# shwetabhardwaj44/EfficientVideoClassification_Youtube8M

Measured on AMD Instinct MI355X. Metric: frames/sec (whole node) H-LSTM teacher+student B=256x300x1152; GAP@20, higher is better.
Workload: dtype bf16; 1 GPU; HierarchicalLstmModel teacher_student every_n=10, lstm_cells=1024x2, MoE(2), batch 256 x 300 x 1152 per GPU; global_batch=256, frames_per_video=300, parallelism=dp1, num_frames=U{120..300}

## Files before the change

### efficientvideoclassification_youtube8m_amd/_lib.py

```python
from __future__ import annotations

import ctypes as C
import os

_HERE = os.path.dirname(os.path.abspath(__file__))
LIB_PATH = os.environ.get("EVC_LIB", os.path.join(_HERE, "libevc_hip.so"))

vp, i32, i64, f32 = C.c_void_p, C.c_int, C.c_int64, C.c_float

SIGNATURES = {
    "evc_check_device": [i32],
    "evc_l2norm_chunk_fwd": [vp, vp, vp, i32, i32, i32, i32, vp, i32, i32, vp, i32, vp, vp, i32, vp, i32, vp, i32, vp],
    "evc_sort_rows_by_len": [vp, i32, i32, vp, vp, vp, vp],
    "evc_frame_counts": [vp, i32, i32, i32, i32, i32, i32, vp, vp, vp, vp],
    "evc_gemm_nt": [vp, i64, vp, i64, vp, i64, i32, i32, i32, vp, i32, i32, vp],
    "evc_gemm_nt_sqnorm": [vp, i64, vp, i64, vp, i64, i32, i32, i32, vp, f32, vp, vp, i64, vp],
    "evc_gemm_tn": [vp, i64, vp, i64, vp, i64, i32, i32, i32, i32, i32, vp],
    "evc_gemm_tn2": [vp, i64, vp, i64, i32, vp, i64, i32, i32, vp, i64, i32, i32, i32, i32, vp],
    "evc_gemm_tn2_rows": [vp, i64, vp, i64, i32, vp, i64, i32, i32, vp, i64, i32, i32, i32, vp, i32, i32, vp],
    "evc_gemm_tn2_slabs": [vp, i64, vp, i64, i32, vp, i64, i32, i32, vp, i64, i64, i32, i32, i32, i32, vp],
    "evc_sum_slabs": [vp, i64, i32, i32, i32, i64, vp, i64, i32, vp],
    "evc_colsum_bf16": [vp, i64, i32, i32, i32, vp, vp],
    "evc_colsum_bf16_det": [vp, i64, i32, i32, i32, vp, vp, i32, vp],
    "evc_lstm_layer_fwd": [vp, vp, vp, vp, i32, i32, i32, i32, i32, vp, vp, vp, vp, i64, vp, vp, vp, vp, vp],
    "evc_lstm_layer_fwd_hp": [vp, vp, i64, vp, i64, vp, vp, i32, i32, i32, i32, vp, vp, vp, vp, vp, i64, vp, vp, vp],
    "evc_gemm_nt_split": [vp, i64, vp, i64, vp, i64, i32, i32, i32, vp, vp],
    "evc_cast_f32_to_f16_wide": [vp, i64, i32, i32, i32, i32, i32, vp, vp],
    "evc_cast_f32_to_bf16_wide": [vp, i64, i32, i32, vp, i64, i32, vp],
    "evc_lstm_layer_fwd_f16": [vp, i64, vp, vp, vp, i32, i32, i32, i32, vp, i32, vp, vp, vp, i64, vp, vp, vp, vp, vp],
    "evc_lstm_layer_fwd_f16_fp8lo": [vp, i64, i32, i64, i32, vp, vp, i32, i32, vp, vp, i32, i32, i32, vp, vp, vp, vp, i64, vp, vp, vp, vp, vp, vp, i32, vp],
    "evc_l2norm_chunk_int": [vp, vp, i32, i32, i32, i32, vp, i32, i32, vp, vp, vp, vp, vp, vp, i32, vp, i32, vp],
    "evc_lstm_level2_fwd_high": [vp, i64, i32, i64, i32, vp, vp, i32, i32, vp, vp, vp, i32, vp, i64, vp, vp, i32, i32, i32, vp, vp, vp, vp, vp, vp, vp, vp, i64,
                                 vp, vp, vp, vp, vp, vp, vp],
    "evc_lstm_layer_fwd_f16_dith": [vp, i64, i32, i64, i32, vp, i64, vp, i64, i32, vp, vp, i32, i32, i32, vp, vp, vp, vp, i64, vp, vp, vp, vp, vp],
    "evc_cast_f32_to_f16_dither": [vp, i64, i32, i64, C.c_uint32, vp, i64, i64, vp],
    "evc_lstm_stack2_fwd_f16_fp8lo": [vp, i32, vp, vp, vp, vp, vp, i32, i32, vp, vp, i32, i32, i32, i32, vp, vp, vp, vp, vp, vp, vp, vp, vp, i64, vp, vp, vp, vp, vp],
    "evc_cast_f32_to_fp8_lo": [vp, i64, i32, i32, i32, i32, i32, vp, i64, vp],
    "evc_cast_f32_to_fp8_lohi": [vp, i64, i32, i32, i32, i32, i32, vp, i64, vp],
    "evc_lstm_layer_bwd": [vp, vp, i32, i32, i32, i32, vp, vp, vp, vp, i64, vp, vp, vp, vp, vp, vp, vp, vp, vp],
    "evc_transpose_to_bf16": [vp, i32, i64, i32, i32, vp, i64, i32, i32, vp],
    "evc_cast_f32_to_bf16": [vp, i64, i32, i32, vp, i64, vp],
    "evc_cast_f32_to_f16": [vp, i64, i32, i32, vp, i64, vp],
    "evc_cast_f32_to_bf16_split": [vp, i64, i32, i32, vp, vp, i64, vp],
    "evc_rowsum_bf16": [vp, i64, i32, i32, vp, vp],
    "evc_lstm_stack2_fwd_f16": [vp, i32, vp, i32, vp, vp, vp, vp, i32, i32, i32, i32, vp, vp, vp, vp, vp, vp, vp, vp, vp, i64, vp, vp, vp, vp, vp],
    "evc_cast_f32_to_f16_segs": [vp, i64, i32, i32, i32, vp, vp],
    "evc_cast_f32_to_f16_wlo": [vp, i64, i32, i32, i32, vp, vp],
    "evc_lstm_level2_fwd": [vp, vp, vp, vp, vp, vp, i32, i32, i32, i32, vp, vp, vp, vp, vp, vp, i64, vp, vp, vp, vp, vp, vp, vp],
# ... 118 lines not shown
```

### efficientvideoclassification_youtube8m_amd/csrc/evc_gemm.hip

```cpp
#include "gemm_shared.h"

template <class Cfg, bool F16 = false, bool FP8 = false>
__global__ __launch_bounds__(Cfg::NT) void gemm_nt_kernel(GemmOperands p, StoreParams s, int tiles_m, int tiles_n) {
  static_assert(!FP8 || (F16 && is_v3<Cfg>::value), "the e4m3 tail rides behind f16 stages of the 64-wide ring loop");
  const int nwg = tiles_m * tiles_n;
  int bid = blockIdx.x, split = 0;
  if (s.splits > 1) {
    split = bid / nwg;
    bid -= split * nwg;
    const int k0 = split * s.ksteps_per_split;
    const int kstep = (is_v2<Cfg>::value && !is_v3<Cfg>::value) ? 32 : 64;
    p.A1 += (long)k0 * kstep;
    p.B += (long)k0 * kstep;
    p.nk1 = min(s.ksteps_per_split, p.nk1 - k0);
    if constexpr (FP8) {
      const int k8 = split * s.ksteps8_per_split;
      p.A3 += (long)k8 * 128;
      p.B8 += (long)k8 * 128;
      p.nk3 = min(s.ksteps8_per_split, p.nk3 - k8);
    }
  }
  const int id = xcd_remap(bid, nwg);
  int tm, tn;
  tile_of(id, tiles_m, tiles_n, tm, tn, s.splits > 1 ? patch_rows(nwg, tiles_n) : 8);
// ... 296 lines not shown
  GemmOperands p;
  p.A1 = (const bf16_t*)A16; p.lda1 = lda; p.nk1 = 0; p.A2 = p.A1; p.lda2 = lda; p.nk2 = 0;
  p.B = (const bf16_t*)B16; p.ldb = ldb; p.group_stride = 0; p.M = M; p.Nu = N;
  p.A1lo = p.A2lo = p.Blo = nullptr;
  p.A3 = A8; p.lda3 = lda8; p.A4 = A8; p.lda4 = lda8; p.B8 = B8; p.ldb8 = ldb8; p.scale8_exp = scale_exp;
  p.amax_ws = amax_ws; p.a8_hi_exp = a8_hi_exp;
  StoreParams s{C, ldc, M, N, bias, 0, 0, 1, 0};
  hipStream_t st = (hipStream_t)stream;
  if (M <= 512) {
    const int tiles = ceil_div(M, 256) * ceil_div(N, 64), nk16 = K16 / 64, nk8 = K8 / 128;
    int splits = 1;
    while (!evc_deterministic() && splits < 16 && tiles * splits * 2 <= 256 && nk16 % (splits * 2) == 0 && nk8 % (splits * 2) == 0 &&
           nk16 / (splits * 2) >= 4 && nk8 / (splits * 2) >= 4)
      splits *= 2;
    if (splits > 1) EVC_CHECK_HIP(hipMemset2DAsync(C, ldc * sizeof(float), 0, (size_t)N * sizeof(float), M, st));
    launch_gemm_f16_fp8<TileCfg3<256, 1, 64, 2, 4, 4>>(p, s, K16, K8, splits, st);
  } else {
    launch_gemm_f16_fp8<TileCfg3<256, 1, 256, 2, 4, 2>>(p, s, K16, K8, 1, st);
  }
  EVC_LAUNCH_CHECK();
  return EVC_OK;
}
extern "C" int evc_gemm_nt_f16_fp8(const evc_f16* A16, int64_t lda, const uint8_t* A8, int64_t lda8, const evc_f16* B16, int64_t ldb,
                                   const uint8_t* B8, int64_t ldb8, float* C, int64_t ldc, int M, int N, int K16, int K8, int scale_exp,
                                   const float* bias, void* stream) {
  return gemm_nt_f16_fp8_impl(A16, lda, A8, lda8, B16, ldb, B8, ldb8, C, ldc, M, N, K16, K8, scale_exp, nullptr, 0, bias, stream);
}
extern "C" int evc_gemm_nt_f16_fp8_dyn(const evc_f16* A16, int64_t lda, const uint8_t* A8, int64_t lda8, const evc_f16* B16, int64_t ldb,
                                       const uint8_t* B8, int64_t ldb8, float* C, int64_t ldc, int M, int N, int K16, int K8, int scale_exp,
                                       const float* amax_ws, int a8_hi_exp, const float* bias, void* stream) {
  EVC_REQUIRE(amax_ws && a8_hi_exp >= -30 && a8_hi_exp <= 30, EVC_ERR_BAD_ARG, "evc_gemm_nt_f16_fp8_dyn: amax_ws=%p a8_hi_exp=%d", (const void*)amax_ws, a8_hi_exp);
  return gemm_nt_f16_fp8_impl(A16, lda, A8, lda8, B16, ldb, B8, ldb8, C, ldc, M, N, K16, K8, scale_exp, amax_ws, a8_hi_exp, bias, stream);
}
```

### efficientvideoclassification_youtube8m_amd/csrc/gemm_core.h

```cpp
#pragma once
#include "evc_common.h"
#include <type_traits>

template <int BM_, int G_, int BU_, int WR_, int WC_>
struct TileCfg {
  static constexpr int BM = BM_, G = G_, BU = BU_, BN = G_ * BU_, WR = WR_, WC = WC_;
  static constexpr int WM = BM / WR, WU = BU / WC, MI = WM / 16, NI = WU / 16;
  static constexpr int NT = 64 * WR * WC;
  static constexpr int BK = 64;
  static constexpr int A_BYTES = BM * 128, B_BYTES = BN * 128, STAGE_BYTES = A_BYTES + B_BYTES;
  static constexpr int LDS_BYTES = 2 * STAGE_BYTES;
  static constexpr int ACH = BM * 8 / NT, BCH = BN * 8 / NT;
  static_assert(WM % 16 == 0 && WU % 16 == 0, "wave tile must be a multiple of 16x16");
  static_assert((BM * 8) % NT == 0 && (BN * 8) % NT == 0, "staging must divide evenly");
};

struct GemmOperands {
  const bf16_t* A1; long lda1; int nk1;
  const bf16_t* A2; long lda2; int nk2;
  const bf16_t* B;  long ldb;
  long group_stride;
  int M;
  int Nu;
  const bf16_t* A1lo; const bf16_t* A2lo; const bf16_t* Blo;
  const bf16_t* B2 = nullptr;
  const uint8_t* A3 = nullptr; long lda3 = 0; int nk3 = 0;
  const uint8_t* A4 = nullptr; long lda4 = 0; int nk4 = 0;
  const uint8_t* B8 = nullptr; long ldb8 = 0;
  int scale8_exp = 0;
  const float* amax_ws = nullptr; int a8_hi_exp = 0;
  const float* row_scale = nullptr; const float* col_add = nullptr; float g2_add = 0.f; long b8_gap = 0;
#ifdef EVC_STAMPS
  int stamp_slot = 0;
#endif
};

__device__ __forceinline__ int xcd_remap(int bid, int nwg) {
  const int xcd = bid & 7, q = nwg >> 3, r = nwg & 7;
  const int base = (xcd < r) ? xcd * (q + 1) : r * (q + 1) + (xcd - r) * q;
  return base + (bid >> 3);
}

__device__ __forceinline__ void tile_of(int id, int tiles_m, int tiles_n, int& tm, int& tn, const int GROUP_M = 8) {
  const int per_group = GROUP_M * tiles_n;
  const int g = id / per_group, r = id - g * per_group;
  const int first_m = g * GROUP_M;
  const int rows = min(tiles_m - first_m, GROUP_M);
  tm = first_m + r % rows;
  tn = r / rows;
}

__device__ __forceinline__ int patch_rows(int nwg, int tiles_n) {
  const int per = max(1, nwg >> 3);
  int gm = 1;
  while (gm * gm * 4 <= per) gm <<= 1;
  while (gm < per && per / gm > tiles_n) gm <<= 1;
  return min(gm, 8);
}

template <class Cfg, bool SWAP = false, bool INIT = true, bool F16 = false>
__device__ __forceinline__ void gemm_mainloop(const GemmOperands& p, const int m0, const int u0, char* lds,
                                              f32x4 (&acc)[Cfg::MI][Cfg::G][Cfg::NI]) {
  const int tid = threadIdx.x;
  const int lane = tid & 63;
// ... 135 lines not shown
```

### efficientvideoclassification_youtube8m_amd/csrc/gemm_core_v2.h

```cpp
#pragma once
#include "gemm_core.h"
#include <type_traits>

constexpr int LOOP_PRODUCER = 1, LOOP_DMA_FIRST = 2, LOOP_NO_PRIO = 4, LOOP_F16 = 8, LOOP_FP8_TAIL = 16;
constexpr int LOOP_B_NT = 64;
constexpr int LOOP_ROW_SCALE = 128;
constexpr int LOOP_MODE_DEFAULT = 0;

template <int BM_, int G_, int BU_, int WR_, int WC_, int STAGES_ = 5, bool PIPE_ = true>
struct TileCfg2 {
  static constexpr int BM = BM_, G = G_, BU = BU_, BN = G_ * BU_, WR = WR_, WC = WC_;
  static constexpr int WM = BM / WR, WU = BU / WC, MI = WM / 16, NI = WU / 16;
  static constexpr int NT = 64 * WR * WC;
  static constexpr int BK = 32, STAGES = STAGES_;
  static constexpr bool PIPE = PIPE_;
  static constexpr int A_BYTES = BM * 64, B_BYTES = BN * 64, STAGE_BYTES = A_BYTES + B_BYTES;
  static constexpr int ACH = (BM * 4 + NT - 1) / NT, BCH = (BN * 4 + NT - 1) / NT;
  static constexpr int PER = ACH + BCH;
  static constexpr bool RAGGED = (BM * 4) % NT != 0 || (BN * 4) % NT != 0;
  static constexpr int DUMMY_OFF = STAGES * STAGE_BYTES;
  static constexpr int LDS_BYTES = DUMMY_OFF + (RAGGED ? 1024 : 0);
  static_assert(WM % 16 == 0 && WU % 16 == 0, "wave tile must be a multiple of 16x16");
  static_assert(BM % 16 == 0 && BN % 16 == 0 && (NT / 4) % 16 == 0, "staging rows per round must keep (row>>2)&3 fixed");
  static_assert(LDS_BYTES <= 160 * 1024, "exceeds the 160 KiB LDS of a CU");
};

__device__ __forceinline__ int swz64(int row) { return (0xD2 >> (2 * ((row >> 2) & 3))) & 3; }

template <int N>
__device__ __forceinline__ void wait_vmcnt() {
  asm volatile("s_waitcnt vmcnt(%0)" ::"n"(N > 63 ? 63 : N) : "memory");
}

template <class Cfg, bool SWAP = false, bool INIT = true, int MODE = LOOP_MODE_DEFAULT>
__device__ __forceinline__ void gemm_mainloop_v2(const GemmOperands& p, const int m0, const int u0, char* lds,
                                                 f32x4 (&acc)[Cfg::MI][Cfg::G][Cfg::NI]) {
  const int tid = threadIdx.x;
  const int lane = tid & 63;
  const int wave = __builtin_amdgcn_readfirstlane(tid >> 6);
// ... 237 lines not shown
```

### efficientvideoclassification_youtube8m_amd/csrc/gemm_core_v3.h

```cpp
#pragma once
#include "gemm_core_v2.h"

#ifdef EVC_STAMPS
static __device__ unsigned long long evc_stamps[8][512][8];
#define EVC_STAMP(slot, k) do { if (threadIdx.x == 0 && blockIdx.x < 512) evc_stamps[(slot) & 7][blockIdx.x][k] = __builtin_amdgcn_s_memrealtime(); } while (0)
#else
#define EVC_STAMP(slot, k) do { } while (0)
#endif
typedef int v4i_t __attribute__((ext_vector_type(4)));
typedef int v8i_t __attribute__((ext_vector_type(8)));

template <int BM_, int G_, int BU_, int WR_, int WC_, int STAGES_ = 4, int MIP_ = 0>
struct TileCfg3 {
  static constexpr int BM = BM_, G = G_, BU = BU_, BN = G_ * BU_, WR = WR_, WC = WC_;
  static constexpr bool UNEVEN = MIP_ > 0;
  static constexpr int MIP = UNEVEN ? MIP_ : BM / WR / 16, MIC = UNEVEN ? BM / 16 - MIP_ : MIP;
  static constexpr int MI = MIP > MIC ? MIP : MIC, WM = UNEVEN ? MI * 16 : BM / WR, ROW1 = UNEVEN ? MIP * 16 : WM;
  static constexpr int WU = BU / WC, NI = WU / 16;
  static_assert(!UNEVEN || (WR == 2 && WC == 4 && BM % 16 == 0 && MIC > 0), "uneven split: two wave rows of four waves (wave row 0 = the producers)");
  static constexpr int NT = 64 * WR * WC;
  static constexpr int BK = 64, STAGES = STAGES_;
  static constexpr bool PIPE = true;
  static constexpr int A_BYTES = BM * 128, B_BYTES = BN * 128, STAGE_BYTES = A_BYTES + B_BYTES;
  static constexpr bool RAGGED = (BM / 8) % (NT / 64) != 0 || (BN / 8) % (NT / 64) != 0 || (BM / 8) % 4 != 0 || (BN / 8) % 4 != 0;
// ... 5 lines not shown
};

template <class Cfg, bool SWAP = false, bool INIT = true, int MODE = LOOP_MODE_DEFAULT, int PHASE = 0>
__device__ __forceinline__ void gemm_mainloop_v3(const GemmOperands& p, const int m0, const int u0, char* lds,
                                                 f32x4 (&acc)[Cfg::MI][Cfg::G][Cfg::NI]) {
  const int tid = threadIdx.x;
  const int lane = tid & 63;
  const int wave = __builtin_amdgcn_readfirstlane(tid >> 6);
  const int wr = wave / Cfg::WC, wc = wave % Cfg::WC;

  if (INIT && PHASE != 1) {
#pragma unroll
    for (int mi = 0; mi < Cfg::MI; ++mi)
#pragma unroll
      for (int g = 0; g < Cfg::G; ++g)
#pragma unroll
        for (int ni = 0; ni < Cfg::NI; ++ni) acc[mi][g][ni] = f32x4{0.f, 0.f, 0.f, 0.f};
  }
  constexpr bool FP8 = (MODE & LOOP_FP8_TAIL) != 0;
  const int nkf = p.nk1 + p.nk2;
  const int nk = nkf + (FP8 ? p.nk3 + p.nk4 : 0);
  if (nk == 0) return;

  const int lc8 = ((lane & 7) ^ (lane >> 3)) * 8;
  constexpr bool PRODUCERS = (MODE & LOOP_PRODUCER) != 0 && Cfg::NT == 512;
  constexpr int NPW = PRODUCERS ? 4 : Cfg::NT / 64;
  const bool producer = wave < NPW;
  constexpr int ACH = (Cfg::BM / 8 + NPW - 1) / NPW, BCH = (Cfg::BN / 8 + NPW - 1) / NPW;
  constexpr int PER = ACH + BCH;
  static_assert(Cfg::RAGGED || (ACH * NPW * 8 == Cfg::BM && BCH * NPW * 8 == Cfg::BN), "surplus pieces need the dummy sink");
  int a_row[ACH];
  uint32_t b_vo[BCH];
  int a_dst[ACH], b_dst[BCH];
#pragma unroll
  for (int i = 0; i < ACH; ++i) {
    const int q = (wave % NPW) + i * NPW;
    const bool live = q < Cfg::BM / 8;
    const int r = live ? q * 8 + (lane >> 3) : 0;
    const int gr = m0 + r;
    a_row[i] = gr < p.M ? gr : p.M - 1;
    a_dst[i] = live ? q * 1024 : -1;
  }
#pragma unroll
  for (int i = 0; i < BCH; ++i) {
    const int q = (wave % NPW) + i * NPW;
    const bool live = q < Cfg::BN / 8;
    const int r = live ? q * 8 + (lane >> 3) : 0;
    const int g = r / Cfg::BU, u = r % Cfg::BU;
    int gu = u0 + u;
    gu = gu < p.Nu ? gu : p.Nu - 1;
    b_vo[i] = FP8 ? (uint32_t)((long)g * p.group_stride + gu) : (uint32_t)((((long)g * p.group_stride + gu) * p.ldb + lc8) * 2);
    b_dst[i] = live ? Cfg::A_BYTES + q * 1024 : -1;
  }
  const bf16_t* const b2 = p.B2 ? p.B2 - (long)p.nk1 * 64 : p.B;
  int ks_issue = 0;
  int slot_issue = 0, slot_read = 0;

  auto stage = [&]() {
    const bool s1 = ks_issue < p.nk1;
    const char* ab = (const char*)(s1 ? p.A1 + (long)ks_issue * 64 : p.A2 + (long)(ks_issue - p.nk1) * 64);
    uint32_t lda_b = (uint32_t)(s1 ? p.lda1 : p.lda2) * 2u;
    const char* b_base = (const char*)((s1 ? p.B : b2) + (long)ks_issue * 64);
    uint32_t ldb_b = (uint32_t)p.ldb * 2u;
    const uint32_t chunk_b = (uint32_t)(lc8 * 2);
    if constexpr (FP8) {
      const int k8 = ks_issue - nkf;
      const bool f = k8 < 0, s3 = k8 < p.nk3;
      const char* ab8 = s3 ? (const char*)p.A3 + (long)k8 * 128 : (const char*)p.A4 + (long)(k8 - p.nk3) * 128;
      ab = f ? ab : ab8;
      lda_b = f ? lda_b : (uint32_t)(s3 ? p.lda3 : p.lda4);
      b_base = f ? b_base : (const char*)p.B8 + (long)k8 * 128 + (s3 ? 0 : p.b8_gap);
      ldb_b = f ? ldb_b : (uint32_t)p.ldb8;
    }
    char* sbase = lds + slot_issue * Cfg::STAGE_BYTES;
#pragma unroll
    for (int i = 0; i < ACH; ++i) {
      char* dst = a_dst[i] >= 0 ? sbase + a_dst[i] : lds + Cfg::DUMMY_OFF;
      const uint32_t vo = __umul24((uint32_t)a_row[i], lda_b) + chunk_b;
      __builtin_amdgcn_global_load_lds((const __attribute__((address_space(1))) void*)(ab + vo),
                                       (__attribute__((address_space(3))) void*)dst, 16, 0, 0);
    }
#pragma unroll
    for (int i = 0; i < BCH; ++i) {
      char* dst = b_dst[i] >= 0 ? sbase + b_dst[i] : lds + Cfg::DUMMY_OFF;
      const uint32_t vo = FP8 ? __umul24(b_vo[i], ldb_b) + chunk_b : b_vo[i];
      __builtin_amdgcn_global_load_lds((const __attribute__((address_space(1))) void*)(b_base + vo),
                                       (__attribute__((address_space(3))) void*)dst, 16, 0, (MODE & LOOP_B_NT) ? 2 : 0);
    }
    ++ks_issue;
    slot_issue = (slot_issue + 1 == Cfg::STAGES) ? 0 : slot_issue + 1;
  };

  const int frow = lane & 15, fq = lane >> 4;
  const int fch = (fq ^ (frow & 7)) * 16;
  const int a_rd0 = (wr * Cfg::ROW1 + frow) * 128 + fch, b_rd0 = Cfg::A_BYTES + (wc * Cfg::WU + frow) * 128 + fch;
  const int a_rd1 = a_rd0 ^ 64, b_rd1 = b_rd0 ^ 64;
  auto a_off = [](const int mi) { return mi * 16 * 128; };
  auto b_off = [](const int g, const int ni) { return (g * Cfg::BU + ni * 16) * 128; };

  auto read_half = [&](auto mi_tag, const int kb, bf16x8 (&af)[Cfg::MI], bf16x8 (&bfr)[Cfg::G][Cfg::NI]) {
    constexpr int MIr = decltype(mi_tag)::value;
    const char* sb = lds + slot_read * Cfg::STAGE_BYTES;
    const char* pa = sb + (kb ? a_rd1 : a_rd0);
    const char* pb = sb + (kb ? b_rd1 : b_rd0);
#pragma unroll
    for (int g = 0; g < Cfg::G; ++g)
#pragma unroll
      for (int ni = 0; ni < Cfg::NI; ++ni) bfr[g][ni] = *(const bf16x8*)(pb + b_off(g, ni));
#pragma unroll
    for (int mi = 0; mi < MIr; ++mi) af[mi] = *(const bf16x8*)(pa + a_off(mi));
  };
  auto next_slot = [&]() { slot_read = (slot_read + 1 == Cfg::STAGES) ? 0 : slot_read + 1; };
  auto mfma_all = [&](auto mi_tag, const bf16x8 (&af)[Cfg::MI], const bf16x8 (&bfr)[Cfg::G][Cfg::NI]) {
#pragma unroll
    for (int mi = 0; mi < decltype(mi_tag)::value; ++mi)
#pragma unroll
      for (int g = 0; g < Cfg::G; ++g)
#pragma unroll
// ... 246 lines not shown
```

### efficientvideoclassification_youtube8m_amd/engine.py

```python
from __future__ import annotations

import math
import os
from collections import OrderedDict

import torch

from . import ops

BF16, F32 = torch.bfloat16, torch.float32


def _align(n, a=16):
    return (n + a - 1) // a * a


def _drain(gen):
    try:
        while True:
            next(gen)
    except StopIteration as e:
        return e.value


# ... 505 lines not shown
                self.x_rows = torch.empty((B, 2 * K), dtype=ops.F16, device=x.device)
            ops.cast_bf16(x, self.x_bf)
            amax = None
            if self.dynamic_fp8_range:
                if not hasattr(self, "x_amax"):
                    self.x_amax = torch.zeros(ops.AMAX_SLOTS, dtype=F32, device=x.device)
                amax = ops.absmax_partials(x, self.x_amax)
            ops.cast_f16_fp8x(x, self.x_rows, amax_ws=amax)
            ops.gemm_nt_f16_fp8(self.x_rows, tw.shadow_w16[self.GATES], tw.shadow_w8[self.GATES], B, V * (Mx + 1), K, self.gate_logits, amax_ws=amax)
            ops.gemm_nt_f16_fp8(self.x_rows, tw.shadow_w16[self.EXPERTS], tw.shadow_w8[self.EXPERTS], B, V * Mx, K, self.expert_logits,
                                bias=tw.store.p(self.EBIAS), amax_ws=amax)
            ops.moe_tail_fwd(self.gate_logits, self.expert_logits, B, V, Mx, self.pred, self.rowsum)
            return self.pred
        if getattr(tw, "precision", "bf16") != "bf16" and hasattr(tw, "shadow_w"):
            if not hasattr(self, "x_w") or self.x_w.shape[0] != B:
                self.x_w = torch.empty((B, 2 * K), dtype=BF16, device=x.device)
            ops.cast_bf16(x, self.x_bf)
            ops.cast_bf16_wide(x, self.x_w, lo_first=True)
            ops.gemm_nt_split_wide(self.x_w, tw.shadow_w[self.GATES], B, V * (Mx + 1), K, self.gate_logits)
            ops.gemm_nt_split_wide(self.x_w, tw.shadow_w[self.EXPERTS], B, V * Mx, K, self.expert_logits, bias=tw.store.p(self.EBIAS))
            ops.moe_tail_fwd(self.gate_logits, self.expert_logits, B, V, Mx, self.pred, self.rowsum)
            return self.pred
        if getattr(tw, "precision", "bf16") != "bf16":
            if not hasattr(self, "x_lo") or self.x_lo.shape != self.x_bf.shape:
                self.x_lo = torch.empty_like(self.x_bf)
            ops.cast_bf16_split(x, self.x_bf, self.x_lo)
            ops.gemm_nt_split(self.x_bf, self.x_lo, tw.shadow_fwd[self.GATES], tw.shadow_lo[self.GATES], B, V * (Mx + 1), K,
                              self.gate_logits)
            ops.gemm_nt_split(self.x_bf, self.x_lo, tw.shadow_fwd[self.EXPERTS], tw.shadow_lo[self.EXPERTS], B, V * Mx, K,
                              self.expert_logits, bias=tw.store.p(self.EBIAS))
            ops.moe_tail_fwd(self.gate_logits, self.expert_logits, B, V, Mx, self.pred, self.rowsum)
            return self.pred
        ops.cast_bf16(x, self.x_bf)
        ops.gemm_nt(self.x_bf, tw.shadow_fwd[self.GATES], B, V * (Mx + 1), K, self.gate_logits)
        ops.gemm_nt(self.x_bf, tw.shadow_fwd[self.EXPERTS], B, V * Mx, K, self.expert_logits,
                    bias=tw.store.p(self.EBIAS))
        ops.moe_tail_fwd(self.gate_logits, self.expert_logits, B, V, Mx, self.pred, self.rowsum)
        return self.pred

    def can_fuse_update(self):
        return (self.V * (self.Mx + 1)) % 4 == 0 and (self.V * self.Mx) % 4 == 0 and self.K % 8 == 0

    dynamic_fp8_range = os.environ.get("EVC_HIGH_DYNAMIC_RANGE", "1") != "0"
    FUSE_MAX_ROWS = 512
    gram_norms = True
    gram_force = None
    skip_stale_fwd_shadow = os.environ.get("EVC_HIGH_KEEP_BF16_SHADOW", "0") != "1"

    @staticmethod
    def gram_slab_count(cols, want):
        if cols <= 0 or cols % 32:
            return 0
        nk = cols // 32
        for S in range(max(1, min(want, nk)), 0, -1):
            if ((nk + S - 1) // S) * (S - 1) < nk:
                return S
        return 0

    def use_gram_norms(self, rows, Vn, cols):
        if not self.gram_norms or self.gram_a is None:
            return False
        K = self.K
        if rows % 32 or rows > 1024 or self.gram_slab_count(K, self.gram_S["x"]) == 0 or self.gram_slab_count(cols, self.gram_S["a"]) == 0:
            return False
        if self.gram_force is not None:
            return self.gram_force
        pass1 = Vn * K * 4.0 / 4.0e12 + 2.0 * rows * Vn * K / 5.0e14
        gram = 42e-6 + 2.0 * rows * rows * (cols + 0.5 * K) / 1.2e14
        return gram < pass1

    def invalidate_norm_cache(self):
        if hasattr(self, "_wsq_valid"):
            self._wsq_valid = [False, False]

    def prefer_fused_update(self, data_parallel):
        return data_parallel or self.B <= self.FUSE_MAX_ROWS

# ... 122 lines not shown
                                        tw.sums[idx[name]], self.partial_ws, clip_norm, lr_t, beta1, beta2, eps, p_wide=wide, p_f16=w16, p_fp8=w8)
                    self._wsq_valid[0 if name == self.GATES else 1] = False
                refreshed_wide = refreshed_wide or wide is not None or w16 is not None
                continue
            self._wsq_valid = [False, False]
            slab = self.slab[name]
            v0 = dp.rank * slab
            vs = min(Vn, v0 + slab) - v0
            args = None
            if vs > 0:
                args = (dlog[:, v0:], x, rows, vs, K, pw[v0:], mw[v0:], vw[v0:], self._full(name)[v0:], tw.shadow_bwd[name][:, v0:],
                        l2, tw.sums[idx[name]], self.partial_ws, clip_norm, lr_t, beta1, beta2, eps)
                ops.moe_grad_update(*args, phase=1)
            dp.all_reduce_small(tw.sums[idx[name]])
            if vs > 0:
                ops.moe_grad_update(*args, phase=2)
            dp.all_gather_slabs(self._full(name), slab)
            sb = tw.shadow_bwd[name]
            ops.transpose_to_bf16(tw.shadow_fwd[name], Vn, K, sb, sb.shape[1])
            self._stale = dp.world > 1
        if tw.precision != "bf16" and not refreshed_wide:
            for name in (self.GATES, self.EXPERTS):
                tw._refresh_high(name)
        gb = st.g(self.EBIAS)
        ops.colsum_bf16(del_, rows, V * Mx, gb)
        ops.grad_sqnorm(gb, None, 0.0, tw.sums[idx[self.EBIAS]])
        ops.clip_adam_step(st.p(self.EBIAS), gb, st.view(st.m, self.EBIAS), st.view(st.v, self.EBIAS), 0.0,
                           tw.sums[idx[self.EBIAS]], clip_norm, lr_t, beta1, beta2, eps)

    def backward(self, dpred, dx_init=None, weight_grads=True, presum_l2=None):
        tw, B, V, Mx, K = self.tw, self.B, self.V, self.Mx, self.K
        ops.moe_tail_bwd(self.gate_logits, self.expert_logits, dpred, B, V, Mx, self.dgl, self.del_)
        V3p, V2p = self.dgl.shape[1], self.del_.shape[1]
        if dx_init is None:
            ops.gemm_nt(self.dgl, tw.shadow_bwd[self.GATES], B, K, V3p, self.dx)
        else:
            self.dx.copy_(dx_init)
            ops.gemm_nt(self.dgl, tw.shadow_bwd[self.GATES], B, K, V3p, self.dx, accumulate=True)
        ops.gemm_nt(self.del_, tw.shadow_bwd[self.EXPERTS], B, K, V2p, self.dx, accumulate=True)
        if not weight_grads:
            return self.dx
        Bp = self.Bp
        ops.transpose_to_bf16(self.dgl, B, V * (Mx + 1), self.dglT, Bp)
        ops.transpose_to_bf16(self.del_, B, V * Mx, self.delT, Bp)
        ops.transpose_to_bf16(self.x_bf, B, K, self.xT, Bp)
        tw._presummed = set()
        for name, aT, Vn in ((self.GATES, self.dglT, V * (Mx + 1)), (self.EXPERTS, self.delT, V * Mx)):
            g = tw.store.g(name)
            if presum_l2 is not None and ops.gemm_nt_sqnorm_ok(Vn, K, Bp) and g.data_ptr() % 16 == 0:
                l2 = presum_l2 if name in tw.l2_names else 0.0
                if getattr(self, "sq_part", None) is None or self.sq_part.numel() < ops.gemm_nt_sqnorm_ws(Vn, K):
                    self.sq_part = torch.empty(ops.gemm_nt_sqnorm_ws(V * (Mx + 1), K), dtype=F32, device=tw.device)
                ops.gemm_nt_sqnorm(aT, self.xT, Vn, K, Bp, g, tw.store.p(name) if l2 else None, l2, tw.sums[list(tw.names).index(name)], ws=self.sq_part)
                tw._presummed.add(name)
            else:
                ops.gemm_nt(aT, self.xT, Vn, K, Bp, g)
        ops.rowsum_bf16(self.delT, V * Mx, Bp, tw.store.g(self.EBIAS))
        return self.dx


class TowerBase:

    l2_names = ()

    def _setup_store(self, shapes, transposed_2d=True):
        self.store = ParamStore(shapes, self.device)
        self.names = list(shapes.keys())
        self.shadow_fwd, self.shadow_bwd = {}, {}
        for k, shp in shapes.items():
            if len(shp) == 2:
                self.shadow_fwd[k] = torch.zeros(shp, dtype=BF16, device=self.device)
                self.shadow_bwd[k] = torch.zeros((shp[1], ops.round_up(shp[0], 64)), dtype=BF16, device=self.device)
# ... 662 lines not shown
```

### efficientvideoclassification_youtube8m_amd/ops.py

```python
from __future__ import annotations

import ctypes as C

import os

import torch

from . import _lib

BF16 = torch.bfloat16
F16 = torch.float16
F32 = torch.float32


def _p(t):
    if t is None:
        return None
    if not t.is_cuda:
        raise _lib.EvcError("evc ops need device tensors (got a CPU tensor); there is no CPU path")
    return t.data_ptr()


def _stream():
    return torch.cuda.current_stream().cuda_stream


MARKS = None


def mark(name):
    if MARKS is not None:
        ev = torch.cuda.Event(enable_timing=True)
        ev.record()
        MARKS.append((name, torch.cuda.current_stream().cuda_stream, ev))


def round_up(x, m):
    return (x + m - 1) // m * m


def check_device(dev=0):
    _lib.call("evc_check_device", dev)


def gemm_nt(A, B, M, N, K, out, bias=None, accumulate=False, lda=None, ldb=None, ldc=None):
    assert A.dtype == BF16 and B.dtype == BF16
    lda = A.stride(0) if lda is None else lda
    ldb = B.stride(0) if ldb is None else ldb
    ldc = out.stride(0) if ldc is None else ldc
    _lib.call("evc_gemm_nt", _p(A), lda, _p(B), ldb, _p(out), ldc, M, N, K, _p(bias),
              1 if out.dtype == BF16 else 0, 1 if accumulate else 0, _stream())
    return out


def _slab_rows_arg(live_rows, K):
    rows, slab = live_rows
    assert slab % 32 == 0 and K == slab * len(rows), (K, slab, len(rows))
    return slab, len(rows), (C.c_int32 * len(rows))(*[int(r) for r in rows])


def gemm_nt_sqnorm(A, B, M, N, K, out, p, l2_coeff, sums, ws=None):
    assert A.dtype == BF16 and B.dtype == BF16 and out.dtype == F32 and out.is_contiguous() and (p is None or (p.dtype == F32 and p.shape == out.shape and p.is_contiguous()))
    need = gemm_nt_sqnorm_ws(M, N)
    if ws is None:
        ws = torch.empty(need, dtype=F32, device=out.device)
    assert ws.dtype == F32 and ws.numel() >= need and ws.is_contiguous()
    _lib.call("evc_gemm_nt_sqnorm", _p(A), A.stride(0), _p(B), B.stride(0), _p(out), out.stride(0), M, N, K, _p(p), float(l2_coeff), _p(sums), _p(ws), ws.numel(),
              _stream())
    return out


def gemm_nt_sqnorm_ws(M, N):
    return 16 * ((M + 127) // 128) * ((N + 127) // 128)


def gemm_nt_sqnorm_ok(M, N, K):
    return M > 512 and N % 256 == 0 and K % 64 == 0 and K < 8192 and os.environ.get("EVC_FUSED_GRAD_NORM", "0") == "1"


def gemm_tn(A, B, M, N, K, out, row_interleave_H=0, accumulate=False, lda=None, ldb=None, ldc=None, live_rows=None):
    assert A.dtype == BF16 and B.dtype == BF16 and out.dtype == F32
    if live_rows is not None:
        slab, ns, arr = _slab_rows_arg(live_rows, K)
        _lib.call("evc_gemm_tn2_rows", _p(A), A.stride(0) if lda is None else lda, _p(B), B.stride(0) if ldb is None else ldb, N, None, 0, 0, 0,
# ... 906 lines not shown
```

### include/evc.h

```cpp
#ifndef EVC_H_
#define EVC_H_

#include <stdint.h>

#ifdef __cplusplus
extern "C" {
#endif

#define EVC_OK 0
#define EVC_ERR_BAD_SHAPE (-1)
#define EVC_ERR_BAD_ALIGN (-2)
#define EVC_ERR_UNSUPPORTED_ARCH (-3)
#define EVC_ERR_HIP (-4)
#define EVC_ERR_BAD_ARG (-5)

#define EVC_VERSION 107

typedef uint16_t evc_bf16;
typedef uint16_t evc_f16;

int evc_version(void);
const char* evc_last_error(void);
int evc_check_device(int dev);

int evc_l2norm_chunk_fwd(const float* x_raw, const uint8_t* x_u8, const int32_t* num_frames,
                         int B, int T, int F,
                         int C1, evc_bf16* out1,
                         int every_n, int C2, evc_bf16* out2, int normalize,
                         evc_bf16* out1_lo, evc_bf16* out2_lo ,
                         int aux_mode ,
                         const int32_t* row_pos1, int rows1, const int32_t* row_pos2, int rows2, void* stream);

int evc_sort_rows_by_len(const int32_t* len, int M, int max_len, int32_t* pos, int32_t* inv, int32_t* len_sorted,
                         void* stream);

int evc_frame_counts(const int32_t* num_frames, int B, int every_n, int subsampled, int max_frames_before_sampling,
                     int num_chunks, int chunk_len, int64_t* n_out, int32_t* len_l1, int32_t* len_l2,
                     void* stream);

int evc_gemm_nt(const evc_bf16* A, int64_t lda, const evc_bf16* B, int64_t ldb, void* C, int64_t ldc,
                int M, int N, int K, const float* bias, int out_bf16, int accumulate, void* stream);
int evc_gemm_nt_sqnorm(const evc_bf16* A, int64_t lda, const evc_bf16* B, int64_t ldb, float* C, int64_t ldc, int M, int N, int K,
                       const float* P, float l2_coeff, float* sums, float* part_ws, int64_t part_ws_floats, void* stream);

int evc_gemm_tn(const evc_bf16* A, int64_t lda, const evc_bf16* B, int64_t ldb, float* C, int64_t ldc,
                int M, int N, int K, int row_interleave_H, int accumulate, void* stream);

int evc_lstm_layer_fwd(const evc_bf16* x, const evc_bf16* wT, const float* bias, const int32_t* len,
                       int T, int M, int Kin, int H, int hoist, float* zx_ws,
                       evc_bf16* hbuf, float* c_state, float* h_state, int64_t ld_state,
                       void* gates, evc_bf16* c_all, const int32_t* row_map, const int32_t* rows_per_step, void* stream);

int evc_lstm_layer_fwd_hp(const evc_bf16* x_lohi, const evc_bf16* wx_hilo, int64_t ldwx, const evc_bf16* wh_hilo, int64_t ldwh,
                          const float* bias, const int32_t* len, int T, int M, int Kin, int H, float* zx_ws,
                          evc_bf16* hbuf, evc_bf16* hbuf_lohi, float* c_state, float* h_state, int64_t ld_state,
                          void* gates, evc_bf16* c_all, void* stream);
int evc_lstm_layer_fwd_f16(const evc_f16* x, int64_t ldx ,
                           const evc_f16* wT, const float* bias, const int32_t* len,
                           int T, int M, int Kin, int H, evc_f16* hbuf,
                           int h_wide ,
                           evc_bf16* hbuf_bf16,
                           float* c_state, float* h_state, int64_t ld_state, void* gates, evc_bf16* c_all,
                           const int32_t* row_map, const int32_t* rows_per_step, void* stream);
int evc_lstm_layer_fwd_f16_fp8lo(const evc_f16* x, int64_t ldx, int kx16, int64_t x8_off, int kx8, const evc_f16* wT16,
                                 const uint8_t* wT8, int w8_scale_exp, int h_lo, const float* bias, const int32_t* len,
                                 int T, int M, int H, evc_f16* hbuf, evc_bf16* hbuf_bf16, float* c_state, float* h_state,
                                 int64_t ld_state, void* gates, evc_bf16* c_all, const int32_t* row_map,
                                 const int32_t* rows_per_step, const float* x_row_scale, const float* x_col_const, int b8_gap, void* stream);
int evc_lstm_layer_fwd_f16_dith(const evc_f16* x, int64_t ldx, int kx16, int64_t x8_off, int kx8, const evc_f16* wT16,
                                int64_t w16_step_stride, const uint8_t* wT8, int64_t ldb8, int scale8_exp, const float* bias,
                                const int32_t* len, int T, int M, int H, evc_f16* hbuf, evc_bf16* hbuf_bf16, float* c_state,
                                float* h_state, int64_t ld_state, void* gates, evc_bf16* c_all, const int32_t* row_map,
                                const int32_t* rows_per_step, void* stream);
int evc_lstm_level2_fwd_high(const evc_f16* x, int64_t ldx, int kx16, int64_t x8_off, int kx8, const evc_f16* wT16_0, const uint8_t* wT8_0,
// ... 275 lines not shown
```

Before: 7.902 million frames/sec.

## Fuse MoE gate/expert GEMMs into single launches for forward and backward

The MoE head's forward now computes both gate and expert logits from the same activations in one kernel launch, splitting the tiles across the two weight matrices. The backward concatenates the two dx products along K (gates and experts) into one split-K kernel with a second B stride, instead of two accumulating GEMMs. This removes launch overhead and a read-modify-write of dx for a small batch-row GEMM, at the cost of new specialised tile configs and atomic split-K accumulation.

Result: no change. 7.965 million frames/sec (median of 6 runs) (+0.8%).

```diff
diff --git a/efficientvideoclassification_youtube8m_amd/_lib.py b/efficientvideoclassification_youtube8m_amd/_lib.py
--- a/efficientvideoclassification_youtube8m_amd/_lib.py
+++ b/efficientvideoclassification_youtube8m_amd/_lib.py
@@ -14,6 +14,8 @@
     "evc_sort_rows_by_len": [vp, i32, i32, vp, vp, vp, vp],
     "evc_frame_counts": [vp, i32, i32, i32, i32, i32, i32, vp, vp, vp, vp],
     "evc_gemm_nt": [vp, i64, vp, i64, vp, i64, i32, i32, i32, vp, i32, i32, vp],
+    "evc_gemm_nt_cols2": [vp, i64, i32, i32, vp, i64, i32, vp, i64, vp, vp, i64, i32, vp, i64, vp, vp],
+    "evc_gemm_nt_k2": [vp, i64, vp, i64, i32, vp, i64, vp, i64, i32, vp, i64, i32, i32, i32, vp],
     "evc_gemm_nt_sqnorm": [vp, i64, vp, i64, vp, i64, i32, i32, i32, vp, f32, vp, vp, i64, vp],
     "evc_gemm_tn": [vp, i64, vp, i64, vp, i64, i32, i32, i32, i32, i32, vp],
     "evc_gemm_tn2": [vp, i64, vp, i64, i32, vp, i64, i32, i32, vp, i64, i32, i32, i32, i32, vp],
diff --git a/efficientvideoclassification_youtube8m_amd/csrc/evc_gemm.hip b/efficientvideoclassification_youtube8m_amd/csrc/evc_gemm.hip
--- a/efficientvideoclassification_youtube8m_amd/csrc/evc_gemm.hip
+++ b/efficientvideoclassification_youtube8m_amd/csrc/evc_gemm.hip
@@ -352,3 +352,160 @@
   EVC_REQUIRE(amax_ws && a8_hi_exp >= -30 && a8_hi_exp <= 30, EVC_ERR_BAD_ARG, "evc_gemm_nt_f16_fp8_dyn: amax_ws=%p a8_hi_exp=%d", (const void*)amax_ws, a8_hi_exp);
   return gemm_nt_f16_fp8_impl(A16, lda, A8, lda8, B16, ldb, B8, ldb8, C, ldc, M, N, K16, K8, scale_exp, amax_ws, a8_hi_exp, bias, stream);
 }
+
+struct Cols2 {
+  const bf16_t* B; long ldb; int N; float* C; long ldc; const float* bias; int tiles1;
+};
+
+template <class Cfg>
+__device__ __forceinline__ void store_tile_rows_f32(f32x4 (&acc)[Cfg::MI][1][Cfg::NI], char* lds, float* C, long ldc, int M, int m0, int u0, const float* bias) {
+  const int lane = threadIdx.x & 63, wave = threadIdx.x >> 6;
+  const int wr = wave / Cfg::WC, wc = wave % Cfg::WC;
+  const int l = lane & 15, g = lane >> 4;
+  constexpr int RS = Cfg::WU * 4 + 16;
+  constexpr int CPR = Cfg::WU / 4, RPI = 64 / CPR, NIT = (Cfg::WM + RPI - 1) / RPI;
+  static_assert(Cfg::WM * RS * (Cfg::NT / 64) <= Cfg::LDS_BYTES, "LDS slice too small for the wave's sub-tile");
+  char* wl = lds + wave * (Cfg::WM * RS);
+  const int colw = u0 + wc * Cfg::WU;
+  const int rbase = m0 + wr * Cfg::WM;
+#pragma unroll
+  for (int ni = 0; ni < Cfg::NI; ++ni) {
+    float4 bv = make_float4(0.f, 0.f, 0.f, 0.f);
+    if (bias) bv = *(const float4*)(bias + colw + ni * 16 + g * 4);
+#pragma unroll
+    for (int mi = 0; mi < Cfg::MI; ++mi) {
+      const f32x4 a = acc[mi][0][ni];
+      *(float4*)(wl + (mi * 16 + l) * RS + (ni * 16 + g * 4) * 4) = make_float4(a[0] + bv.x, a[1] + bv.y, a[2] + bv.z, a[3] + bv.w);
+    }
+  }
+  asm volatile("s_waitcnt lgkmcnt(0)" ::: "memory");
+  const int rsub = lane / CPR, c16 = (lane - rsub * CPR) * 16;
+#pragma unroll
+  for (int it = 0; it < NIT; ++it) {
+    const int rl = it * RPI + rsub;
+    const int row = rbase + rl;
+    if (rsub < RPI && rl < Cfg::WM && row < M) {
+      const uint4 q = *(const uint4*)(wl + rl * RS + c16);
+      *(uint4*)((char*)(C + (long)row * ldc + colw) + c16) = q;
+    }
+  }
+}
+
+template <class Cfg, int XMODE>
+__global__ __launch_bounds__(Cfg::NT) void gemm_rows_kernel(GemmOperands p, StoreParams s, Cols2 c2, int tiles_n) {
+  static_assert(is_v3<Cfg>::value && Cfg::G == 1, "batch-row products run on the 64-wide ring stages");
+  int bid = blockIdx.x, split = 0;
+  if (s.splits > 1) {
+    split = bid / tiles_n;
+    bid -= split * tiles_n;
+    const int k0 = split * s.ksteps_per_split, k1 = min(k0 + s.ksteps_per_split, p.nk1 + p.nk2);
+    const int a0 = min(k0, p.nk1), a1 = min(k1, p.nk1);
+    const int b0 = max(k0, p.nk1) - p.nk1, b1 = max(k1, p.nk1) - p.nk1;
+    p.A1 += (long)a0 * 64; p.B += (long)a0 * 64; p.nk1 = a1 - a0;
+    p.A2 += (long)b0 * 64; p.nk2 = b1 - b0;
+    if (p.B2) p.B2 += (long)b0 * 64;
+  }
+  int tn = xcd_remap(bid, tiles_n);
+  if (tn >= c2.tiles1) {
+    tn -= c2.tiles1;
+    p.B = c2.B; p.ldb = c2.ldb; p.Nu = c2.N;
+    s.C = c2.C; s.ldc = c2.ldc; s.N = c2.N; s.bias = c2.bias;
+  }
+  const int m0 = 0, u0 = tn * Cfg::BU;
+  f32x4 acc[Cfg::MI][1][Cfg::NI];
+  run_mainloop<Cfg, 1, true, true, LOOP_PRODUCER | LOOP_DMA_FIRST | LOOP_NO_PRIO | LOOP_B_NT | XMODE>(p, m0, u0, acc);
+  if constexpr (64 % Cfg::WU == 0) {
+    if (s.splits > 1) {
+      __syncthreads();
+      store_tile_via_lds<Cfg, 4, true>(acc, lds_dyn, s.C, s.ldc, s.M, s.N, m0, u0, split == 0 ? s.bias : nullptr);
+      return;
+    }
+  }
+  const bool via_lds = s.splits == 1 && !s.accumulate && (s.ldc * 4) % 16 == 0 && ((uintptr_t)s.C % 16) == 0 && (!s.bias || ((uintptr_t)s.bias % 16) == 0);
+  if (via_lds) {
+    const int wc = (threadIdx.x >> 6) % Cfg::WC;
+    __syncthreads();
+    if (u0 + wc * Cfg::WU + Cfg::WU <= s.N) {
+      store_tile_rows_f32<Cfg>(acc, lds_dyn, (float*)s.C, s.ldc, s.M, m0, u0, s.bias);
+      return;
+    }
+  }
+  TileCoordsT<Cfg> tc;
+#pragma unroll
+  for (int mi = 0; mi < Cfg::MI; ++mi) {
+    const int m = m0 + tc.row0 + mi * 16;
+    if (m >= s.M) continue;
+#pragma unroll
+    for (int ni = 0; ni < Cfg::NI; ++ni)
+#pragma unroll
+      for (int r = 0; r < 4; ++r) {
+        const int n = u0 + tc.unit0 + ni * 16 + r;
+        if (n >= s.N) continue;
+        float v = acc[mi][0][ni][r] + ((s.bias && split == 0) ? s.bias[n] : 0.f);
+        float* cp = (float*)s.C + (long)m * s.ldc + n;
+        if (s.splits > 1) {
+          atomicAdd(cp, v);
+        } else {
+          if (s.accumulate) v += *cp;
+          *cp = v;
+        }
+      }
+  }
+}
+
+typedef TileCfg3<256, 1, 96, 4, 2, 3> CfgRows96;
+typedef TileCfg3<256, 1, 64, 2, 4, 4> CfgRows64;
+
+extern "C" int evc_gemm_nt_cols2(const evc_bf16* A, int64_t lda, int M, int K,
+                                 const evc_bf16* B1, int64_t ldb1, int N1, float* C1, int64_t ldc1, const float* bias1,
+                                 const evc_bf16* B2, int64_t ldb2, int N2, float* C2, int64_t ldc2, const float* bias2, void* stream) {
+  EVC_REQUIRE(M > 0 && M <= 256 && N1 > 0 && N2 > 0 && K >= 64 && K % 64 == 0, EVC_ERR_BAD_SHAPE,
+              "evc_gemm_nt_cols2: bad shape M=%d (1..256) N1=%d N2=%d K=%d (%%64)", M, N1, N2, K);
+  EVC_REQUIRE(A && B1 && B2 && C1 && C2, EVC_ERR_BAD_ARG, "evc_gemm_nt_cols2: NULL operand");
+  EVC_REQUIRE(lda % 8 == 0 && ldb1 % 8 == 0 && ldb2 % 8 == 0 && lda >= K && ldb1 >= K && ldb2 >= K && ldc1 >= N1 && ldc2 >= N2 &&
+              ((uintptr_t)A % 16) == 0 && ((uintptr_t)B1 % 16) == 0 && ((uintptr_t)B2 % 16) == 0, EVC_ERR_BAD_ALIGN,
+              "evc_gemm_nt_cols2: operands must be 16-byte aligned (lda=%ld ldb1=%ld ldb2=%ld)", (long)lda, (long)ldb1, (long)ldb2);
+  EVC_REQUIRE(ring_operand_ok(M, lda) && ring_operand_ok(N1, ldb1) && ring_operand_ok(N2, ldb2), EVC_ERR_BAD_SHAPE,
+              "evc_gemm_nt_cols2: an operand spans 4 GiB or more");
+  typedef CfgRows96 Cfg;
+  GemmOperands p;
+  p.A1 = A; p.lda1 = lda; p.nk1 = K / 64; p.A2 = A; p.lda2 = lda; p.nk2 = 0;
+  p.B = B1; p.ldb = ldb1; p.group_stride = 0; p.M = M; p.Nu = N1;
+  p.A1lo = p.A2lo = p.Blo = nullptr;
+  StoreParams s{C1, ldc1, M, N1, bias1, 0, 0, 1, p.nk1};
+  const int t1 = ceil_div(N1, Cfg::BU), t2 = ceil_div(N2, Cfg::BU);
+  Cols2 c2{B2, ldb2, N2, C2, ldc2, bias2, t1};
+  launch_cfg<Cfg>(gemm_rows_kernel<Cfg, 0>, t1 + t2, (hipStream_t)stream, p, s, c2, t1 + t2);
+  EVC_LAUNCH_CHECK();
+  return EVC_OK;
+}
+
+extern "C" int evc_gemm_nt_k2(const evc_bf16* A1, int64_t lda1, const evc_bf16* B1, int64_t ldb1, int K1,
+                              const evc_bf16* A2, int64_t lda2, const evc_bf16* B2, int64_t ldb2, int K2,
+                              float* C, int64_t ldc, int M, int N, int accumulate, void* stream) {
+  EVC_REQUIRE(M > 0 && M <= 256 && N > 0 && K1 >= 64 && K1 % 64 == 0 && K2 >= 64 && K2 % 64 == 0, EVC_ERR_BAD_SHAPE,
+              "evc_gemm_nt_k2: bad shape M=%d (1..256) N=%d K1=%d K2=%d (%%64, >= 64)", M, N, K1, K2);
+  EVC_REQUIRE(A1 && B1 && A2 && B2 && C, EVC_ERR_BAD_ARG, "evc_gemm_nt_k2: NULL operand");
+  EVC_REQUIRE(lda1 % 8 == 0 && ldb1 % 8 == 0 && lda2 % 8 == 0 && ldb2 % 8 == 0 && lda1 >= K1 && ldb1 >= K1 && lda2 >= K2 && ldb2 >= K2 && ldc >= N &&
+              ((uintptr_t)A1 % 16) == 0 && ((uintptr_t)B1 % 16) == 0 && ((uintptr_t)A2 % 16) == 0 && ((uintptr_t)B2 % 16) == 0, EVC_ERR_BAD_ALIGN,
+              "evc_gemm_nt_k2: operands must be 16-byte aligned (lda1=%ld ldb1=%ld lda2=%ld ldb2=%ld)", (long)lda1, (long)ldb1, (long)lda2, (long)ldb2);
+  EVC_REQUIRE(ring_operand_ok(M, lda1) && ring_operand_ok(M, lda2) && ring_operand_ok(N, ldb1) && ring_operand_ok(N, ldb2), EVC_ERR_BAD_SHAPE,
+              "evc_gemm_nt_k2: an operand spans 4 GiB or more");
+  typedef CfgRows64 Cfg;
+  GemmOperands p;
+  p.A1 = A1; p.lda1 = lda1; p.nk1 = K1 / 64; p.A2 = A2; p.lda2 = lda2; p.nk2 = K2 / 64;
+  p.B = B1; p.ldb = ldb1; p.B2 = B2; p.ldb2 = ldb2; p.group_stride = 0; p.M = M; p.Nu = N;
+  p.A1lo = p.A2lo = p.Blo = nullptr;
+  const int tn = ceil_div(N, Cfg::BU), nk = p.nk1 + p.nk2;
+  int splits = 256 / tn;
+  if (splits > (K1 + K2) / 1024) splits = (K1 + K2) / 1024;
+  if (splits < 1 || evc_deterministic()) splits = 1;
+  while (splits > 1 && (long)ceil_div(nk, splits) * (splits - 1) >= nk) --splits;
+  hipStream_t st = (hipStream_t)stream;
+  if (splits > 1 && !accumulate) EVC_CHECK_HIP(hipMemset2DAsync(C, ldc * sizeof(float), 0, (size_t)N * sizeof(float), M, st));
+  StoreParams s{C, ldc, M, N, nullptr, 0, accumulate, splits, ceil_div(nk, splits)};
+  Cols2 c2{nullptr, 0, 0, nullptr, 0, nullptr, tn};
+  launch_cfg<Cfg>(gemm_rows_kernel<Cfg, LOOP_B2_LD>, tn * splits, st, p, s, c2, tn);
+  EVC_LAUNCH_CHECK();
+  return EVC_OK;
+}
diff --git a/efficientvideoclassification_youtube8m_amd/csrc/gemm_core.h b/efficientvideoclassification_youtube8m_amd/csrc/gemm_core.h
--- a/efficientvideoclassification_youtube8m_amd/csrc/gemm_core.h
+++ b/efficientvideoclassification_youtube8m_amd/csrc/gemm_core.h
@@ -30,6 +30,7 @@
   int scale8_exp = 0;
   const float* amax_ws = nullptr; int a8_hi_exp = 0;
   const float* row_scale = nullptr; const float* col_add = nullptr; float g2_add = 0.f; long b8_gap = 0;
+  long ldb2 = 0;
 #ifdef EVC_STAMPS
   int stamp_slot = 0;
 #endif
diff --git a/efficientvideoclassification_youtube8m_amd/csrc/gemm_core_v2.h b/efficientvideoclassification_youtube8m_amd/csrc/gemm_core_v2.h
--- a/efficientvideoclassification_youtube8m_amd/csrc/gemm_core_v2.h
+++ b/efficientvideoclassification_youtube8m_amd/csrc/gemm_core_v2.h
@@ -5,6 +5,7 @@
 constexpr int LOOP_PRODUCER = 1, LOOP_DMA_FIRST = 2, LOOP_NO_PRIO = 4, LOOP_F16 = 8, LOOP_FP8_TAIL = 16;
 constexpr int LOOP_B_NT = 64;
 constexpr int LOOP_ROW_SCALE = 128;
+constexpr int LOOP_B2_LD = 256;
 constexpr int LOOP_MODE_DEFAULT = 0;
 
 template <int BM_, int G_, int BU_, int WR_, int WC_, int STAGES_ = 5, bool PIPE_ = true>
diff --git a/efficientvideoclassification_youtube8m_amd/csrc/gemm_core_v3.h b/efficientvideoclassification_youtube8m_amd/csrc/gemm_core_v3.h
--- a/efficientvideoclassification_youtube8m_amd/csrc/gemm_core_v3.h
+++ b/efficientvideoclassification_youtube8m_amd/csrc/gemm_core_v3.h
@@ -61,6 +61,8 @@
   int a_row[ACH];
   uint32_t b_vo[BCH];
   int a_dst[ACH], b_dst[BCH];
+  constexpr bool B2LD = (MODE & LOOP_B2_LD) != 0;
+  static_assert(!B2LD || !FP8, "LOOP_B2_LD: 16-bit stages only");
 #pragma unroll
   for (int i = 0; i < ACH; ++i) {
     const int q = (wave % NPW) + i * NPW;
@@ -78,7 +80,7 @@
     const int g = r / Cfg::BU, u = r % Cfg::BU;
     int gu = u0 + u;
     gu = gu < p.Nu ? gu : p.Nu - 1;
-    b_vo[i] = FP8 ? (uint32_t)((long)g * p.group_stride + gu) : (uint32_t)((((long)g * p.group_stride + gu) * p.ldb + lc8) * 2);
+    b_vo[i] = (FP8 || B2LD) ? (uint32_t)((long)g * p.group_stride + gu) : (uint32_t)((((long)g * p.group_stride + gu) * p.ldb + lc8) * 2);
     b_dst[i] = live ? Cfg::A_BYTES + q * 1024 : -1;
   }
   const bf16_t* const b2 = p.B2 ? p.B2 - (long)p.nk1 * 64 : p.B;
@@ -90,7 +92,7 @@
     const char* ab = (const char*)(s1 ? p.A1 + (long)ks_issue * 64 : p.A2 + (long)(ks_issue - p.nk1) * 64);
     uint32_t lda_b = (uint32_t)(s1 ? p.lda1 : p.lda2) * 2u;
     const char* b_base = (const char*)((s1 ? p.B : b2) + (long)ks_issue * 64);
-    uint32_t ldb_b = (uint32_t)p.ldb * 2u;
+    uint32_t ldb_b = (uint32_t)((B2LD && !s1) ? p.ldb2 : p.ldb) * 2u;
     const uint32_t chunk_b = (uint32_t)(lc8 * 2);
     if constexpr (FP8) {
       const int k8 = ks_issue - nkf;
@@ -112,7 +114,7 @@
 #pragma unroll
     for (int i = 0; i < BCH; ++i) {
       char* dst = b_dst[i] >= 0 ? sbase + b_dst[i] : lds + Cfg::DUMMY_OFF;
-      const uint32_t vo = FP8 ? __umul24(b_vo[i], ldb_b) + chunk_b : b_vo[i];
+      const uint32_t vo = (FP8 || B2LD) ? __umul24(b_vo[i], ldb_b) + chunk_b : b_vo[i];
       __builtin_amdgcn_global_load_lds((const __attribute__((address_space(1))) void*)(b_base + vo),
                                        (__attribute__((address_space(3))) void*)dst, 16, 0, (MODE & LOOP_B_NT) ? 2 : 0);
     }
diff --git a/efficientvideoclassification_youtube8m_amd/engine.py b/efficientvideoclassification_youtube8m_amd/engine.py
--- a/efficientvideoclassification_youtube8m_amd/engine.py
+++ b/efficientvideoclassification_youtube8m_amd/engine.py
@@ -561,9 +561,13 @@
             ops.moe_tail_fwd(self.gate_logits, self.expert_logits, B, V, Mx, self.pred, self.rowsum)
             return self.pred
         ops.cast_bf16(x, self.x_bf)
-        ops.gemm_nt(self.x_bf, tw.shadow_fwd[self.GATES], B, V * (Mx + 1), K, self.gate_logits)
-        ops.gemm_nt(self.x_bf, tw.shadow_fwd[self.EXPERTS], B, V * Mx, K, self.expert_logits,
-                    bias=tw.store.p(self.EBIAS))
+        if self.one_launch and B <= 256 and K % 64 == 0:
+            ops.gemm_nt_cols2(self.x_bf, tw.shadow_fwd[self.GATES], tw.shadow_fwd[self.EXPERTS], B, V * (Mx + 1), V * Mx, K,
+                              self.gate_logits, self.expert_logits, bias2=tw.store.p(self.EBIAS))
+        else:
+            ops.gemm_nt(self.x_bf, tw.shadow_fwd[self.GATES], B, V * (Mx + 1), K, self.gate_logits)
+            ops.gemm_nt(self.x_bf, tw.shadow_fwd[self.EXPERTS], B, V * Mx, K, self.expert_logits,
+                        bias=tw.store.p(self.EBIAS))
         ops.moe_tail_fwd(self.gate_logits, self.expert_logits, B, V, Mx, self.pred, self.rowsum)
         return self.pred
 
@@ -572,6 +576,7 @@
 
     dynamic_fp8_range = os.environ.get("EVC_HIGH_DYNAMIC_RANGE", "1") != "0"
     FUSE_MAX_ROWS = 512
+    one_launch = True
     gram_norms = True
     gram_force = None
     skip_stale_fwd_shadow = os.environ.get("EVC_HIGH_KEEP_BF16_SHADOW", "0") != "1"
@@ -760,12 +765,18 @@
         tw, B, V, Mx, K = self.tw, self.B, self.V, self.Mx, self.K
         ops.moe_tail_bwd(self.gate_logits, self.expert_logits, dpred, B, V, Mx, self.dgl, self.del_)
         V3p, V2p = self.dgl.shape[1], self.del_.shape[1]
-        if dx_init is None:
-            ops.gemm_nt(self.dgl, tw.shadow_bwd[self.GATES], B, K, V3p, self.dx)
+        if self.one_launch and B <= 256 and getattr(tw, "precision", "bf16") == "bf16" and not ops.DETERMINISTIC:
+            if dx_init is not None:
+                self.dx.copy_(dx_init)
+            ops.gemm_nt_k2(self.dgl, tw.shadow_bwd[self.GATES], V3p, self.del_, tw.shadow_bwd[self.EXPERTS], V2p, B, K, self.dx,
+                           accumulate=dx_init is not None)
         else:
-            self.dx.copy_(dx_init)
-            ops.gemm_nt(self.dgl, tw.shadow_bwd[self.GATES], B, K, V3p, self.dx, accumulate=True)
-        ops.gemm_nt(self.del_, tw.shadow_bwd[self.EXPERTS], B, K, V2p, self.dx, accumulate=True)
+            if dx_init is None:
+                ops.gemm_nt(self.dgl, tw.shadow_bwd[self.GATES], B, K, V3p, self.dx)
+            else:
+                self.dx.copy_(dx_init)
+                ops.gemm_nt(self.dgl, tw.shadow_bwd[self.GATES], B, K, V3p, self.dx, accumulate=True)
+            ops.gemm_nt(self.del_, tw.shadow_bwd[self.EXPERTS], B, K, V2p, self.dx, accumulate=True)
         if not weight_grads:
             return self.dx
         Bp = self.Bp
diff --git a/efficientvideoclassification_youtube8m_amd/ops.py b/efficientvideoclassification_youtube8m_amd/ops.py
--- a/efficientvideoclassification_youtube8m_amd/ops.py
+++ b/efficientvideoclassification_youtube8m_amd/ops.py
@@ -50,6 +50,20 @@
     ldc = out.stride(0) if ldc is None else ldc
     _lib.call("evc_gemm_nt", _p(A), lda, _p(B), ldb, _p(out), ldc, M, N, K, _p(bias),
               1 if out.dtype == BF16 else 0, 1 if accumulate else 0, _stream())
+    return out
+
+
+def gemm_nt_cols2(A, B1, B2, M, N1, N2, K, out1, out2, bias1=None, bias2=None):
+    assert A.dtype == BF16 and B1.dtype == BF16 and B2.dtype == BF16 and out1.dtype == F32 and out2.dtype == F32
+    _lib.call("evc_gemm_nt_cols2", _p(A), A.stride(0), M, K, _p(B1), B1.stride(0), N1, _p(out1), out1.stride(0), _p(bias1),
+              _p(B2), B2.stride(0), N2, _p(out2), out2.stride(0), _p(bias2), _stream())
+    return out1, out2
+
+
+def gemm_nt_k2(A1, B1, K1, A2, B2, K2, M, N, out, accumulate=False):
+    assert A1.dtype == BF16 and B1.dtype == BF16 and A2.dtype == BF16 and B2.dtype == BF16 and out.dtype == F32
+    _lib.call("evc_gemm_nt_k2", _p(A1), A1.stride(0), _p(B1), B1.stride(0), K1, _p(A2), A2.stride(0), _p(B2), B2.stride(0), K2,
+              _p(out), out.stride(0), M, N, 1 if accumulate else 0, _stream())
     return out
 
 
diff --git a/include/evc.h b/include/evc.h
--- a/include/evc.h
+++ b/include/evc.h
@@ -40,6 +40,12 @@
 
 int evc_gemm_nt(const evc_bf16* A, int64_t lda, const evc_bf16* B, int64_t ldb, void* C, int64_t ldc,
                 int M, int N, int K, const float* bias, int out_bf16, int accumulate, void* stream);
+int evc_gemm_nt_cols2(const evc_bf16* A, int64_t lda, int M, int K,
+                      const evc_bf16* B1, int64_t ldb1, int N1, float* C1, int64_t ldc1, const float* bias1,
+                      const evc_bf16* B2, int64_t ldb2, int N2, float* C2, int64_t ldc2, const float* bias2, void* stream);
+int evc_gemm_nt_k2(const evc_bf16* A1, int64_t lda1, const evc_bf16* B1, int64_t ldb1, int K1,
+                   const evc_bf16* A2, int64_t lda2, const evc_bf16* B2, int64_t ldb2, int K2,
+                   float* C, int64_t ldc, int M, int N, int accumulate, void* stream);
 int evc_gemm_nt_sqnorm(const evc_bf16* A, int64_t lda, const evc_bf16* B, int64_t ldb, float* C, int64_t ldc, int M, int N, int K,
                        const float* P, float l2_coeff, float* sums, float* part_ws, int64_t part_ws_floats, void* stream);
 
```
